# CUAI/Edge-Proposal-Sets

Measured on AMD Instinct MI355X. Metric: candidate edges scored/sec on ogbl-ppa (ppa-like synthetic): Adamic-Adar over the FULL 2-hop non-edge candidate set + top-4M selection, higher is better.
Workload: dtype int64

## Files before the change

edge-proposal-sets_amd/csrc/scan_pieces.hip:

```cpp
#include "eps_common.h"
#include "scan_common.h"
#include <string.h>
#include <atomic>

#define SP_EMPTY 0u
#define SP_MAXP (SP_M + 1)
#define SP_UBITS 8192
#define SP_SB 4
#define SP_PACKED_X8 8u
#define SP_MODE_RATIO 2270u
#define SP_MODE_RATIO_WIDE 8000u
#define SP_BATCH 8
#define SP_G 1
#define SP_LEAN_ROWS 256
#define SP_LEAN_T 256
#define SP_LEAN_G 2
#define SP_LEAN_CHUNK 2048u

typedef short sp_v2s __attribute__((ext_vector_type(2)));

typedef unsigned short sp_v2us __attribute__((ext_vector_type(2)));

struct sp_unit {
    v4i u4;
    v4f a4;
    uint32_t fx;
    int nvalid;
};

template <class Emit>
__device__ __forceinline__ int sp_plan_column(const sp_params &p, int32_t v, int32_t dv, int lane, int32_t my_bound, uint32_t pwk,
                                              int32_t nbk, uint32_t direct_ids, Emit emit)
{
    const uint32_t ek = (uint32_t)eps_wave_incl_scan_dpp((int)pwk) - pwk;
    const bool pk_on = p.ssum != nullptr;
    const uint32_t sv = pk_on ? p.ssum[v] - (p.heads ? (p.heads[v].y < p.ssum[v] ? p.heads[v].y : p.ssum[v]) : 0u) : 0u;
    const uint32_t smk = pk_on ? p.smax[lane <= SP_M ? lane : SP_M] : 0u;
    const int kv = __popcll(__ballot(lane >= 1 && lane < SP_M && my_bound <= v - 1));
    const int32_t hi_k = my_bound < v ? my_bound : v;
    int np = 0, k0 = 0;
    while (k0 <= kv) {
        const int32_t lo = __builtin_amdgcn_readlane(my_bound, k0);
        const uint32_t e0 = (uint32_t)__builtin_amdgcn_readlane((int)ek, k0);
        const bool in = lane > k0 && lane <= kv + 1;
        const int kd = k0 + __popcll(__ballot(in && (uint32_t)(hi_k - lo) <= direct_ids));
        const int32_t nb0 = __builtin_amdgcn_readlane(nbk, k0);
        const int kh = k0 + __popcll(__ballot(in && (ek - e0) + (uint32_t)(nbk - nb0) <= p.piece_paths));
        int kp = k0, kd16 = k0;
        uint32_t ms = 0u;
        if (pk_on) {
            const uint32_t sm0 = (uint32_t)__builtin_amdgcn_readlane((int)smk, k0);
            ms = sv < sm0 ? sv : sm0;
            const uint32_t need_s = (ms >> p.packed_dmax) + (uint32_t)dv + 2u;
            if (need_s < 0x7FFFu) kd16 = k0 + __popcll(__ballot(in && (uint32_t)(hi_k - lo) <= 2u * direct_ids));
            const uint32_t span = (uint32_t)(hi_k - lo);
            const int kb = 32 - __clz((int)((span > 2u ? span : 2u) - 1u));
            const uint32_t cap = kb >= 30 ? 0u : (1u << (31 - kb)) - 1u;
            kp = k0 + __popcll(__ballot(in && (ek - e0) + (uint32_t)(nbk - nb0) <= p.packed_paths && need_s < cap));
            if (p.wide_paths && dv <= p.wide_rows) {
                const int kw = k0 + __popcll(__ballot(in && (ek - e0) <= p.wide_paths));
                kp = kw > kp ? kw : kp;
            }
        }
        int k1;
        uint32_t flag = 0u, pq = 0u;
        const int kdd = kd16 > kd ? kd16 : kd;
        bool take_direct = kdd >= kh && kdd >= kp && kdd > k0;
        if (!take_direct && kdd > k0 && kp > kdd && kp >= kh) {
            const uint32_t pd = (uint32_t)__builtin_amdgcn_readlane((int)ek, kdd) - e0;
            const uint32_t pp = (uint32_t)__builtin_amdgcn_readlane((int)ek, kp) - e0;
            take_direct = (unsigned long long)(pp - pd) * p.mode_ratio < (unsigned long long)pd * pp;
        }
        if (take_direct && kd16 > kd) {
            k1 = kd16;
            flag = 0xC0000000u;
            uint32_t d = 0u;
            while ((ms >> d) + (uint32_t)dv + 2u >= 0x7FFFu) ++d;
            pq = d | (16u << 8);
        } else if (take_direct) {
            k1 = kd;
            flag = 0x80000000u;
        } else if (kp >= kh && kp > k0) {
            k1 = kp;
            flag = 0x40000000u;
            const uint32_t span = (uint32_t)(__builtin_amdgcn_readlane(hi_k, k1) - lo);
            const int kb = 32 - __clz((int)((span > 2u ? span : 2u) - 1u));
            if (p.wide_paths && dv <= p.wide_rows) {
                pq = (uint32_t)(kb < 31 ? kb : 31) << 8;
            } else {
                const uint32_t cap = (1u << (31 - kb)) - 1u;
                uint32_t d = 0u;
                while ((ms >> d) + (uint32_t)dv + 2u >= cap) ++d;
                pq = d | ((uint32_t)kb << 8);
            }
        } else if (kh > k0) {
            k1 = kh;
        } else {
            k1 = k0 + 1;
        }
        const uint32_t sum = (uint32_t)__builtin_amdgcn_readlane((int)ek, k1) - e0;
        if (sum) {
            emit(np, k0, k1, lo, __builtin_amdgcn_readlane(hi_k, k1), sum | flag, pq, __builtin_amdgcn_readlane(nbk, k0),
                 __builtin_amdgcn_readlane(nbk, k1));
            ++np;
        }
        k0 = k1;
    }
    return np;
}

template <int T, bool HV, bool FULL, bool PACK, bool SK = false, bool LEAN = false>
__global__ __launch_bounds__(T, 4) void scan_piece_kernel(sp_params p)
{
    static_assert(!LEAN || (!HV && FULL && PACK && SK), "the lean body serves the main launch's tables only");
    constexpr int G = LEAN ? SP_LEAN_G : SP_G;
    constexpr int ROWS = LEAN ? SP_LEAN_ROWS : T;
    extern __shared__ __attribute__((aligned(16))) uint32_t lds[];
    const int slots = 1 << p.table_bits;
    uint32_t *tkey = lds;
    uint32_t *tval = lds + slots;
    uint4 *r_desc = (uint4 *)(lds + 2 * slots);
    uint32_t *ubits = lds + ((2 * slots + 4 * (ROWS + 1) + 3) & ~3);
    uint16_t *wrank = (uint16_t *)(ubits + SP_UBITS / 32);
    __shared__ unsigned long long s_alloc;
    __shared__ int s_rbase;
    __shared__ int32_t s_pk0[SP_MAXP], s_pk1[SP_MAXP];
    __shared__ int32_t s_plo[SP_MAXP], s_phi[SP_MAXP];
    __shared__ uint32_t s_pinfo[SP_MAXP];
    __shared__ uint32_t s_pq[SP_MAXP];
    __shared__ int32_t s_pna[SP_MAXP], s_pnb[SP_MAXP];
    __shared__ int s_np;
    __shared__ unsigned int s_ticket;
    __shared__ unsigned int s_out_cur, s_out_end;
    __shared__ unsigned int s_fill_lo, s_fill_hi;
    __shared__ unsigned long long s_ncand;
    __shared__ unsigned int s_hot;
    __shared__ uint32_t s_em[SP_EM];

    const int tid = threadIdx.x, lane = tid & 63;
    const int wib = __builtin_amdgcn_readfirstlane(tid >> 6);
    const uint32_t out_cap = p.out->capacity;
    int64_t *__restrict__ out_key = p.out->key;
    float *__restrict__ out_val = p.out->val;
    const uint32_t *__restrict__ rowptr_lo = (const uint32_t *)p.rowptr;
    const __amdgpu_buffer_rsrc_t col_rs = eps_raw_rsrc(p.col, p.col_bytes);
    const __amdgpu_buffer_rsrc_t val_rs = eps_raw_rsrc(HV ? (const void *)p.val : (const void *)p.col, p.col_bytes);
    const uint32_t thr32 = sp_bar_units(p.out->threshold, p.shift, HV);
    const uint32_t direct_ids = 2u * (uint32_t)slots;
    const bool no_bar = !FULL && thr32 <= 1u;
    const bool raw_sums = FULL || p.heads != nullptr;
    const uint32_t chunk = LEAN ? SP_LEAN_CHUNK : no_bar && direct_ids > 8192u ? direct_ids : 8192u;
    const int32_t my_bound = p.bounds[lane <= SP_M ? lane : SP_M];
    if (LEAN && thr32 >= SP_FLAG) {
        if (tid == 0) atomicOr(p.status, 2u);
        return;
    }

    for (int i = tid; i < 2 * slots; i += T) lds[i] = 0u;
    for (int i = tid; i < SP_UBITS / 32; i += T) ubits[i] = 0u;
    for (int i = tid; i < SP_EM; i += T) s_em[i] = 0u;
    if (tid == 0) {
        s_out_cur = 0u;
        s_out_end = 0u;
        s_fill_lo = 0u;
        s_fill_hi = 0u;
        s_alloc = 0ull;
        s_ncand = 0ull;
    }
    bool sketch_seen = false;
    const unsigned int ncol = (unsigned int)p.n_columns;
    const unsigned int batch_from = p.batch_from;
    auto first_of = [&](unsigned int tk) { return tk < batch_from ? tk : batch_from + (tk - batch_from) * SP_BATCH; };
    unsigned int t = blockIdx.x < batch_from ? blockIdx.x : first_of(blockIdx.x);
    unsigned int t_end = t + (blockIdx.x < batch_from ? 1u : SP_BATCH);
    eps_lds_barrier();

    while (t < ncol) {
        const bool last_of_ticket = t + 1u >= t_end || t + 1u >= ncol;
        unsigned int t_next = 0;
        if (tid == 0 && last_of_ticket) t_next = gridDim.x + atomicAdd(p.next_col, 1u);
        int32_t v, dv;
        uint32_t vb;
        uint4 cra = make_uint4(0u, 0u, 0u, 0u), crb = make_uint4(0u, 0u, 0u, 0u);
        if (FULL || p.colrec) {
            cra = p.colrec[2 * (size_t)t];
            crb = p.colrec[2 * (size_t)t + 1];
            v = (int32_t)cra.x;
            vb = cra.y;
            dv = (int32_t)cra.z;
        } else {
            v = p.columns[t];
            vb = rowptr_lo[2 * (size_t)v];
            dv = (int32_t)(rowptr_lo[2 * (size_t)v + 2] - vb);
        }
        const int32_t *__restrict__ vcol = p.col + vb;
        const int32_t *__restrict__ vrev = p.revpos + vb;
        const int rounds = LEAN ? 1 : (dv + T - 1) / T;
        const bool single = LEAN || rounds == 1;
        uint32_t xv = 0u, thr_v = thr32;
        bool bad_head = false;
        if (FULL || p.heads) {
            const uint2 hd = (FULL || p.colrec) ? make_uint2(cra.w, crb.x) : p.heads[v];
            xv = hd.x;
            if (thr32 < SP_FLAG) {
                bad_head = hd.y >= thr32;
                thr_v = thr32 - hd.y;
            }
            if (bad_head && tid == 0) atomicOr(p.status, 4u);
            if ((FULL || p.ssum) && thr32 < SP_FLAG && ((FULL || p.colrec) ? crb.y : p.ssum[v]) < thr32) bad_head = true;
        }
        if (LEAN && dv > ROWS) {
            if (tid == 0) atomicOr(p.status, 2u);
            bad_head = true;
        }
        if (dv > 0 && v > 0 && !bad_head) {
            uint32_t my_w = 0, my_rev = 0, my_base = 0, my_fx = 0;
            uint32_t cut_first = 0u;
            if (PACK && single && tid < dv) {
                const uint4 pa = p.pack[2 * ((size_t)vb + (size_t)tid)];
                my_w = pa.x;
                my_base = pa.y;
                my_fx = pa.z;
                my_rev = pa.w & 0xFFFFu;
                cut_first = pa.w >> 16;
            }
            if (!PACK && single && tid < dv) {
                my_w = (uint32_t)vcol[tid];
                my_rev = (uint32_t)vrev[tid];
            }
            if (!PACK && single && tid < dv) {
                my_base = (FULL || p.rowrec) ? p.rowrec[(size_t)my_w * 32 + 16] : rowptr_lo[2 * (size_t)my_w];
                my_fx = HV ? __builtin_bit_cast(uint32_t, (p.val[vb + tid] * p.node_w[my_w]) * p.up)
                           : ((FULL || p.rowrec) ? p.rowrec[(size_t)my_w * 32 + 17] : p.fx32[my_w]);
            }
            if (!FULL && wib == 0 && !p.plan) {
                const uint32_t pwk = lane < SP_M ? p.wpaths[(size_t)v * SP_M + lane] : 0u;
                const int32_t nbk = lane >= 1 && lane <= SP_M ? (int32_t)p.cuts[(size_t)v * SP_M + lane - 1] : 0;
                const int np = sp_plan_column(p, v, dv, lane, my_bound, pwk, nbk, direct_ids,
                                              [&](int i, int k0, int k1, int32_t lo, int32_t hi, uint32_t info, uint32_t pq, int32_t na, int32_t nb) {
                                                  if (lane == 0) {
                                                      s_pk0[i] = k0;
                                                      s_pk1[i] = k1;
                                                      s_plo[i] = lo;
                                                      s_phi[i] = hi;
                                                      s_pinfo[i] = info;
                                                      s_pq[i] = pq;
                                                      s_pna[i] = na;
                                                      s_pnb[i] = nb;
                                                  }
                                              });
                if (lane == 0) s_np = np;
            } else if (FULL || p.plan) {
                const uint32_t pb = (FULL || p.colrec) ? crb.z : p.pptr[v];
                const int np = (FULL || p.colrec) ? (int)crb.w : (int)(p.pptr[v + 1] - pb);
                if (tid < np) {
                    const uint4 rec = p.plan[pb + (uint32_t)tid];
                    const int k1 = (int)((rec.y >> 8) & 0xFFu);
                    const int32_t bk = p.bounds[k1];
                    s_pinfo[tid] = rec.x;
                    s_pk0[tid] = (int)(rec.y & 0xFFu);
                    s_pk1[tid] = k1;
                    s_pq[tid] = rec.y >> 16;
                    s_pna[tid] = (int32_t)(rec.z & 0xFFFFu);
                    s_pnb[tid] = (int32_t)(rec.z >> 16);
                    s_plo[tid] = (int32_t)rec.w;
                    s_phi[tid] = bk < v ? bk : v;
                }
                if (tid == 0) s_np = np;
            }
            eps_lds_barrier();
            const int np = s_np;
            uint32_t cut_ahead = 0u, seg_from = 0u;
            const uint16_t *__restrict__ cut_tab = (FULL || p.rowrec) ? (const uint16_t *)p.rowrec : p.cuts;
            const size_t cut_ld = (FULL || p.rowrec) ? 64u : (size_t)SP_M;
            const uint16_t *__restrict__ pack16 = (const uint16_t *)p.pack;
            if (PACK) cut_ahead = cut_first;
            else if (single && tid < dv && np > 0) cut_ahead = cut_tab[(size_t)my_w * cut_ld + s_pk1[0] - 1];

            for (int pi = 0; pi < np; ++pi) {
                const int k0 = s_pk0[pi], k1 = s_pk1[pi];
                const int na = s_pna[pi], nb = s_pnb[pi];
                const uint32_t info = s_pinfo[pi];
                if (LEAN && (info >> 30) == 0u) {
                    if (tid == 0) atomicOr(p.status, 2u);
                    continue;
                }
                const bool direct = (info >> 31) != 0u;
                const bool d16 = !HV && (info >> 30) == 3u;
                const bool packed_kind = !HV && (info >> 30) == 1u;
                const bool sketch = LEAN ? packed_kind : SK && packed_kind && single && p.sketch != 0u && thr_v < SP_FLAG;
                const bool packed = !LEAN && packed_kind && !sketch;
                const bool quant = packed || d16;
                const uint32_t ppaths = info & 0x3FFFFFFFu;
                const uint32_t pq = quant ? s_pq[pi] : 0u;
                const uint32_t pk_d = pq & 0xFFu, pk_sb = quant ? 32u - (pq >> 8) : 16u;
                const uint32_t pk_flag = quant ? 1u << (pk_sb - 1u) : 0u;
                const uint32_t pk_thr = thr_v >= SP_FLAG ? 0xFFFFFFFFu : ((thr_v >> pk_d) ? (thr_v >> pk_d) : 1u);
                const int32_t lo_id = s_plo[pi], hi_id = s_phi[pi];
                const uint32_t pkeys = ppaths + (uint32_t)(nb - na);
                int plog = 0;
                if (!LEAN && !direct && !packed && !sketch && pkeys > p.piece_paths) {
                    const uint32_t q = (pkeys + p.piece_paths - 1u) / p.piece_paths;
                    plog = 32 - __clz((int)(q - 1u)) + 1;
                }
                const uint32_t parts = LEAN ? 1u : 1u << plog;
                int bits;
                {
                    const uint32_t per = (pkeys + parts - 1u) >> plog;
                    const int max_bits = packed || sketch ? p.table_bits + 1 : p.table_bits;
                    const int want = per > 1u ? 33 - __clz((int)(per - 1u)) : 1;
                    bits = want < 10 ? 10 : (want > max_bits ? max_bits : want);
                }
                const uint32_t mask = (1u << bits) - 1u;
                const uint32_t span = (uint32_t)(hi_id - lo_id);
                const uint32_t scan_slots = d16 ? (span + 1u) >> 1 : direct ? span : (1u << bits);
                const uint32_t cand_max = direct ? span : (1u << bits);
                if (tid == 0) {
                    s_hot = 0u;
                    uint32_t need = ppaths < cand_max ? ppaths : cand_max;
                    if (!no_bar && need > 1024u) need = 1024u;
                    if (need > chunk) need = chunk;
                    const uint32_t left = s_out_cur < s_out_end ? s_out_end - s_out_cur : 0u;
                    if (left < need) {
                        s_fill_lo = s_out_cur < out_cap ? s_out_cur : out_cap;
                        s_fill_hi = left ? (s_out_end < out_cap ? s_out_end : out_cap) : s_fill_lo;
                        const unsigned long long b64 = atomicAdd(&p.out->count, (unsigned long long)chunk);
                        const uint32_t b = b64 < (unsigned long long)out_cap ? (uint32_t)b64 : out_cap;
                        s_out_cur = b;
                        s_out_end = b + chunk;
                    }
                }
                uint32_t seg_a = 0u, seg_len = 0u;
                if (single && tid < dv) {
                    const uint32_t b = cut_ahead < my_rev ? cut_ahead : my_rev;
                    seg_a = seg_from;
                    seg_len = (uint32_t)tid < xv ? 0u : b - seg_from;
                    seg_from = b;
                    if (pi + 1 < np)
                        cut_ahead = PACK && pi + 1 <= 8 ? pack16[((size_t)vb + (size_t)tid) * 16 + 7 + (pi + 1)]
                                                        : cut_tab[(size_t)my_w * cut_ld + s_pk1[pi + 1] - 1];
                }
                auto emit = [&](uint32_t u, uint32_t sum) {
                    uint32_t pos = atomicAdd(&s_out_cur, 1u);
                    if (pos >= s_out_end) {
                        const unsigned long long q = atomicAdd(&p.out->count, 1ull);
                        pos = q < (unsigned long long)out_cap ? (uint32_t)q : out_cap;
                    }
                    if (pos < out_cap) {
                        out_key[pos] = ((int64_t)v << 32) | (int64_t)u;
                        out_val[pos] = raw_sums ? __builtin_bit_cast(float, sum) : (float)sum * p.scale;
                    }
                };
                for (uint32_t part = 0; part < parts; ++part) {
                    uint32_t new_keys = 0u;
                    for (int j = sketch ? nb : single ? tid : na + tid; j < nb; j += T) {
                        const uint32_t u = single ? my_w : (uint32_t)vcol[j];
                        if (j >= na && (int32_t)u >= lo_id && (int32_t)u < hi_id) {
                            if (d16) {
                                const uint32_t o = u - (uint32_t)lo_id;
                                atomicOr(&lds[o >> 1], 0x8000u << ((o & 1u) << 4));
                            } else if (direct) {
                                lds[u - (uint32_t)lo_id] = SP_FLAG;
                            } else if (packed) {
                                const uint32_t mix = sp_mix(u);
                                uint32_t h = mix >> (32 - bits);
                                const uint32_t st = ((mix >> 7) | 1u) & mask;
                                const uint32_t word = ((u - (uint32_t)lo_id) << pk_sb) | pk_flag;
                                for (uint32_t tries = 0; tries <= mask; ++tries) {
                                    if (atomicCAS(&lds[h], 0u, word) == 0u) break;
                                    h = (h + st) & mask;
                                }
                            } else if (!LEAN) {
                                const uint32_t mix = sp_mix(u);
                                if ((mix & (parts - 1u)) == part) {
                                    uint32_t h = mix >> (32 - bits);
                                    const uint32_t st = ((mix >> 7) | 1u) & mask;
                                    for (uint32_t tries = 0; tries <= mask; ++tries) {
                                        if (atomicCAS(&tkey[h], SP_EMPTY, u + 1u) == SP_EMPTY) {
                                            tval[h] = SP_FLAG;
                                            break;
                                        }
                                        h = (h + st) & mask;
                                    }
                                }
                            }
                        }
                    }
                    for (int r = 0; r < rounds; ++r) {
                        const int j = r * T + tid;
                        uint32_t w = my_w, rev = my_rev, base = my_base, fx = my_fx;
                        uint32_t len = 0u, a = 0u;
                        if (single) {
                            a = seg_a;
                            len = seg_len;
                        } else if (j < dv) {
                            w = (uint32_t)vcol[j];
                            rev = (uint32_t)vrev[j];
                            base = (FULL || p.rowrec) ? p.rowrec[(size_t)w * 32 + 16] : rowptr_lo[2 * (size_t)w];
                            fx = HV ? __builtin_bit_cast(uint32_t, (p.val[vb + j] * p.node_w[w]) * p.up)
                                    : ((FULL || p.rowrec) ? p.rowrec[(size_t)w * 32 + 17] : p.fx32[w]);
                            const uint16_t *crow = cut_tab + (size_t)w * cut_ld;
                            uint32_t b = crow[k1 - 1];
                            if (k0 > 0) a = crow[k0 - 1];
                            a = a < rev ? a : rev;
                            b = b < rev ? b : rev;
                            len = (uint32_t)j < xv ? 0u : b - a;
                        }
                        const int units = (int)((len + 3u) >> 2);
                        const int flag = units > 0 ? 1 : 0;
                        const int incl_c = eps_wave_incl_scan_dpp(units | (flag << 24));
                        const int incl = incl_c & 0xFFFFFF, incl_f = (int)((uint32_t)incl_c >> 24);
                        unsigned long long got = 0ull;
                        if (lane == 63) got = atomicAdd(&s_alloc, ((unsigned long long)(uint32_t)incl << 32) | (unsigned long long)(uint32_t)incl_f);
                        const int woff = __builtin_amdgcn_readlane((int)(got >> 32), 63);
                        const int woff_f = __builtin_amdgcn_readlane((int)(uint32_t)got, 63);
                        const uint32_t a_u = (uint32_t)(incl - units + woff);
                        if (flag) {
                            const int d = incl_f - 1 + woff_f;
                            r_desc[d] = make_uint4(base + a, len, quant ? (fx + ((1u << pk_d) - 1u)) >> pk_d : fx, a_u);
                            if (a_u < (uint32_t)SP_UBITS) atomicOr(&ubits[a_u >> 5], 1u << (a_u & 31u));
                        }
                        eps_lds_barrier();
                        if (s_fill_hi > s_fill_lo) {
                            const uint32_t f0 = s_fill_lo, f1 = s_fill_hi;
                            for (uint32_t i = f0 + (uint32_t)tid; i < f1; i += T) {
                                out_key[i] = -1;
                                out_val[i] = -__builtin_inff();
                            }
                        }
                        int total = (int)(s_alloc >> 32);
                        if (LEAN && total > SP_UBITS) {
                            if (tid == 0) atomicOr(p.status, 2u);
                            total = SP_UBITS;
                        }
                        for (uint32_t ulo = 0; ulo < (uint32_t)total && (!LEAN || ulo == 0u); ulo += SP_UBITS) {
                            const uint32_t uhi = ulo + SP_UBITS < (uint32_t)total ? ulo + SP_UBITS : (uint32_t)total;
                            if (ulo > 0u) {
                                for (int i = tid; i < SP_UBITS / 32; i += T) ubits[i] = 0u;
                                if (tid == 0) s_rbase = 0;
                                eps_lds_barrier();
                                const unsigned long long before = __ballot(flag && a_u + (uint32_t)units <= ulo);
                                if (lane == 0 && before) atomicAdd(&s_rbase, __popcll(before));
                                if (flag && a_u + (uint32_t)units > ulo && a_u < uhi) {
                                    const uint32_t pos = (a_u > ulo ? a_u : ulo) - ulo;
                                    atomicOr(&ubits[pos >> 5], 1u << (pos & 31));
                                }
                                eps_lds_barrier();
                            }
                            const int rbase = ulo > 0u ? s_rbase : 0;
                            {
                                const uint4 b4 = *(const uint4 *)(ubits + 4 * lane);
                                const int c0 = __popc(b4.x), c1 = c0 + __popc(b4.y), c2 = c1 + __popc(b4.z), c3 = c2 + __popc(b4.w);
                                const int ex = eps_wave_incl_scan_dpp(c3) - c3;
                                uint2 pk;
                                pk.x = (uint32_t)ex | ((uint32_t)(ex + c0) << 16);
                                pk.y = (uint32_t)(ex + c1) | ((uint32_t)(ex + c2) << 16);
                                *(uint2 *)(wrank + 4 * lane) = pk;
                                asm volatile("s_waitcnt lgkmcnt(0)" ::: "memory");
                            }
                        auto fetch_group = [&](int it0, sp_unit (&f)[G]) {
                            int lo[G];
#pragma unroll
                            for (int q = 0; q < G; ++q) {
                                const uint32_t sr = (uint32_t)((it0 + q) * T + tid);
                                const uint32_t wd = sr < SP_UBITS ? sr >> 5 : 0u;
                                const uint32_t bits = ubits[wd];
                                const int rk = (int)wrank[wd];
                                lo[q] = rbase + rk + __popc(bits & ((2u << (sr & 31u)) - 1u)) - 1;
                                lo[q] = lo[q] < 0 ? 0 : lo[q];
                            }
#pragma unroll
                            for (int q = 0; q < G; ++q) {
                                const int s = (int)ulo + (it0 + q) * T + tid;
// ... 107 lines not shown
                                        }
                                    }
                                    if (++tries > 4u * (mask + 2u)) {
                                        if (have || pend) atomicOr(p.status, 2u);
                                        have = false;
                                        pend = 0u;
                                    }
                                }
                            } else if (!LEAN) {
                                constexpr int E = 4 * G;
                                uint32_t key[E], h[E], mixv[E];
                                uint32_t pend = 0u;
#pragma unroll
                                for (int q = 0; q < G; ++q) pend |= ((1u << f[q].nvalid) - 1u) << (4 * q);
#pragma unroll
                                for (int i = 0; i < E; ++i) {
                                    const uint32_t id = (uint32_t)f[i >> 2].u4[i & 3];
                                    mixv[i] = sp_mix(id);
                                    key[i] = id + 1u;
                                    h[i] = mixv[i] >> (32 - bits);
                                }
                                if (parts > 1u) {
#pragma unroll
                                    for (int i = 0; i < E; ++i)
                                        if ((mixv[i] & (parts - 1u)) != part) pend &= ~(1u << i);
                                }
                                uint32_t old[E], pfx[E];
#pragma unroll
                                for (int i = 0; i < E; ++i) pfx[i] = path_fx(f[i >> 2], i & 3);
#pragma unroll
                                for (int i = 0; i < E; ++i)
                                    if (pend & (1u << i)) old[i] = atomicCAS(&tkey[h[i]], SP_EMPTY, key[i]);
#pragma unroll
                                for (int i = 0; i < E; ++i)
                                    if ((pend & (1u << i)) && (old[i] == SP_EMPTY || old[i] == key[i])) {
                                        atomicAdd(&tval[h[i]], pfx[i]);
                                        pend &= ~(1u << i);
                                        new_keys += old[i] == SP_EMPTY ? 1u : 0u;
                                    }
                                uint32_t ch = 0u, cstep = 0u, ckey = 0u, cfx = 0u, tries = 0u;
                                bool have = false;
                                while (__ballot(have || pend != 0u)) {
                                    if (!have && pend != 0u) {
                                        const int e = __ffs((int)pend) - 1;
                                        pend &= pend - 1u;
                                        uint32_t m = mixv[0];
                                        ch = h[0];
                                        ckey = key[0];
                                        cfx = pfx[0];
#pragma unroll
                                        for (int i = 1; i < E; ++i)
                                            if (e == i) {
                                                m = mixv[i];
                                                ch = h[i];
                                                ckey = key[i];
                                                cfx = pfx[i];
                                            }
                                        cstep = ((m >> 7) | 1u) & mask;
                                        have = true;
                                    }
                                    if (have) {
                                        ch = (ch + cstep) & mask;
                                        const uint32_t o = atomicCAS(&tkey[ch], SP_EMPTY, ckey);
                                        if (o == SP_EMPTY || o == ckey) {
                                            atomicAdd(&tval[ch], cfx);
                                            new_keys += o == SP_EMPTY ? 1u : 0u;
                                            have = false;
                                        }
                                    }
                                    if (++tries > 4u * (mask + 2u)) {
                                        if (have || pend) atomicOr(p.status, 2u);
                                        have = false;
                                        pend = 0u;
                                    }
                                }
                            }
                        };
                        {
                            const int n_iter = (int)(uhi - ulo + T - 1) / T;
                            sp_unit fa[G], fb[G];
                            fetch_group(0, fa);
                            if (n_iter <= G) {
                                consume_group(fa);
                            } else {
                                for (int it0 = 0; it0 < n_iter; it0 += 2 * G) {
                                    fetch_group(it0 + G, fb);
                                    consume_group(fa);
                                    fetch_group(it0 + 2 * G, fa);
                                    consume_group(fb);
                                }
                            }
                        }
                        if (sketch) {
                            if (tid == 0 && !sketch_seen) atomicOr(p.status, 16u);
                            sketch_seen = true;
                            eps_lds_barrier();
                            const uint32_t half = 1u << (bits - 1);
                            {
                                uint32_t mx = 0u;
                                for (uint32_t i = 4u * (uint32_t)tid; i < half; i += 4u * T) {
                                    const uint4 a4 = *(const uint4 *)(lds + i);
                                    const uint32_t m01 = a4.x > a4.y ? a4.x : a4.y, m23 = a4.z > a4.w ? a4.z : a4.w;
                                    const uint32_t m = m01 > m23 ? m01 : m23;
                                    mx = m > mx ? m : mx;
                                }
                                if (__ballot(mx >= thr_v) && lane == 0) s_hot = 1u;
                            }
                            eps_lds_barrier();
                            if (s_hot) {
                            const int n_iter = (int)(uhi - ulo + T - 1) / T;
                            auto report = [&](uint32_t u, uint32_t est) {
                                int a = na, b = nb;
                                while (a < b) {
                                    const int mid = (a + b) >> 1;
                                    if (vcol[mid] < (int32_t)u) a = mid + 1; else b = mid;
                                }
                                if (a < nb && vcol[a] == (int32_t)u) return;
                                const uint32_t em_mask = (p.sketch >> 1 ? p.sketch >> 1 : (uint32_t)SP_EM) - 1u;
                                uint32_t h = (sp_mix(u) >> 9) & em_mask;
                                for (uint32_t tries = 0; tries <= em_mask; ++tries) {
                                    const uint32_t old = atomicCAS(&s_em[h], 0u, u + 1u);
                                    if (old == 0u) {
                                        emit(u, est);
                                        return;
                                    }
                                    if (old == u + 1u) return;
                                    h = (h + 1u) & em_mask;
                                }
                                atomicOr(p.status, 8u);
                            };
                            auto look = [&](const sp_unit (&f)[G]) {
                                uint32_t est[4 * G];
#pragma unroll
                                for (int i = 0; i < 4 * G; ++i) {
                                    const uint32_t id = (uint32_t)f[i >> 2].u4[i & 3];
                                    const uint32_t ea = lds[sp_mix(id) >> (33 - bits)], eb = lds[half + (sp_mix2(id) >> (33 - bits))];
                                    est[i] = ea < eb ? ea : eb;
                                }
#pragma unroll
                                for (int i = 0; i < 4 * G; ++i)
                                    if ((i & 3) < f[i >> 2].nvalid && est[i] >= thr_v) report((uint32_t)f[i >> 2].u4[i & 3], est[i]);
                            };
                            sp_unit fa[G], fb[G];
                            fetch_group(0, fa);
                            if (n_iter <= G) {
                                look(fa);
                            } else {
                                for (int it0 = 0; it0 < n_iter; it0 += 2 * G) {
                                    fetch_group(it0 + G, fb);
                                    look(fa);
                                    fetch_group(it0 + 2 * G, fa);
                                    look(fb);
                                }
                            }
                            }
                        }
                            if (!LEAN && uhi < (uint32_t)total) eps_lds_barrier();
                        }
                        eps_lds_barrier();
                        for (int i = tid; i < SP_UBITS / 32; i += T) ubits[i] = 0u;
                        if (tid == 0) {
                            s_alloc = 0ull;
                            s_fill_hi = 0u;
                        }
                        if (r + 1 < rounds) eps_lds_barrier();
                    }
                    const int thr_s = thr_v >= SP_FLAG ? 0x7FFFFFFF : (int)thr_v;
                    if (d16) {
                        const int thr_h = pk_thr >= 0x8000u ? 0x7FFFFFFF : (int)(pk_thr << 16);
                        sp_v2us pc16 = (sp_v2us)(0);
                        uint32_t ones = 0x00010001u;
                        asm("" : "+v"(ones));
                        const uint32_t n4 = (scan_slots + 3u) & ~3u;
                        for (uint32_t i0 = 0; i0 < n4; i0 += 4u * SP_SB * T) {
                            uint4 s4[SP_SB];
#pragma unroll
                            for (int b = 0; b < SP_SB; ++b) {
                                const uint32_t i = i0 + 4u * T * b + 4u * tid;
                                s4[b] = i < n4 ? *(const uint4 *)(lds + i) : make_uint4(0u, 0u, 0u, 0u);
                            }
#pragma unroll
                            for (int b = 0; b < SP_SB; ++b) {
                                const uint32_t i = i0 + 4u * T * b + 4u * tid;
                                if (i < n4) *(uint4 *)(lds + i) = make_uint4(0u, 0u, 0u, 0u);
                                const uint32_t wv[4] = {s4[b].x, s4[b].y, s4[b].z, s4[b].w};
#pragma unroll
                                for (int e = 0; e < 4; ++e) {
                                    const sp_v2s pos = __builtin_elementwise_max(__builtin_bit_cast(sp_v2s, wv[e]), (sp_v2s)(0));
                                    pc16 += __builtin_elementwise_min(__builtin_bit_cast(sp_v2us, pos), __builtin_bit_cast(sp_v2us, ones));
                                }
                                int x[8];
#pragma unroll
                                for (int e = 0; e < 4; ++e) {
                                    x[2 * e] = (int)(wv[e] << 16);
                                    x[2 * e + 1] = (int)(wv[e] & 0xFFFF0000u);
                                }
                                int m = x[0];
#pragma unroll
                                for (int e = 1; e < 8; ++e) m = x[e] > m ? x[e] : m;
                                if (m >= thr_h) {
#pragma unroll
                                    for (int e = 0; e < 8; ++e)
                                        if (x[e] >= thr_h) emit((uint32_t)lo_id + 2u * i + e, ((uint32_t)x[e] >> 16) << pk_d);
                                }
                            }
                        }
                        new_keys += (uint32_t)pc16.x + (uint32_t)pc16.y;
                    } else if (direct) {
                        const uint32_t n4 = (scan_slots + 3u) & ~3u;
                        for (uint32_t i0 = 0; i0 < n4; i0 += 4u * SP_SB * T) {
                            uint4 s4[SP_SB];
#pragma unroll
                            for (int b = 0; b < SP_SB; ++b) {
                                const uint32_t i = i0 + 4u * T * b + 4u * tid;
                                s4[b] = i < n4 ? *(const uint4 *)(lds + i) : make_uint4(0u, 0u, 0u, 0u);
                            }
#pragma unroll
                            for (int b = 0; b < SP_SB; ++b) {
                                const uint32_t i = i0 + 4u * T * b + 4u * tid;
                                if (i < n4) *(uint4 *)(lds + i) = make_uint4(0u, 0u, 0u, 0u);
                                const int sv[4] = {(int)s4[b].x, (int)s4[b].y, (int)s4[b].z, (int)s4[b].w};
#pragma unroll
                                for (int e = 0; e < 4; ++e) new_keys += sv[e] > 0 ? 1u : 0u;
                                const int m01 = sv[0] > sv[1] ? sv[0] : sv[1], m23 = sv[2] > sv[3] ? sv[2] : sv[3];
                                if ((m01 > m23 ? m01 : m23) >= thr_s) {
#pragma unroll
                                    for (int e = 0; e < 4; ++e)
                                        if (sv[e] >= thr_s) emit((uint32_t)lo_id + i + e, (uint32_t)sv[e]);
                                }
                            }
                        }
                    } else if (sketch) {
                        for (uint32_t i = 4u * (uint32_t)tid; i < scan_slots; i += 4u * T) *(uint4 *)(lds + i) = make_uint4(0u, 0u, 0u, 0u);
                        for (int i = tid; i < SP_EM; i += T) s_em[i] = 0u;
                    } else if (packed) {
                        const uint32_t kb = 32u - pk_sb;
                        const int thr_p = pk_thr >= pk_flag ? 0x7FFFFFFF : (int)(pk_thr << kb);
                        for (uint32_t i0 = 0; i0 < scan_slots; i0 += 4u * SP_SB * T) {
                            uint4 s4[SP_SB];
#pragma unroll
                            for (int b = 0; b < SP_SB; ++b) {
                                const uint32_t i = i0 + 4u * T * b + 4u * tid;
                                s4[b] = i < scan_slots ? *(const uint4 *)(lds + i) : make_uint4(0u, 0u, 0u, 0u);
                            }
#pragma unroll
                            for (int b = 0; b < SP_SB; ++b) {
                                const uint32_t i = i0 + 4u * T * b + 4u * tid;
                                if (i < scan_slots) *(uint4 *)(lds + i) = make_uint4(0u, 0u, 0u, 0u);
                                const uint32_t sv[4] = {s4[b].x, s4[b].y, s4[b].z, s4[b].w};
                                const int x[4] = {(int)(sv[0] << kb), (int)(sv[1] << kb), (int)(sv[2] << kb), (int)(sv[3] << kb)};
                                const int m01 = x[0] > x[1] ? x[0] : x[1], m23 = x[2] > x[3] ? x[2] : x[3];
                                if ((m01 > m23 ? m01 : m23) >= thr_p) {
#pragma unroll
                                    for (int e = 0; e < 4; ++e)
                                        if (x[e] >= thr_p) emit((uint32_t)lo_id + (sv[e] >> pk_sb), ((uint32_t)x[e] >> kb) << pk_d);
                                }
                            }
                        }
                    } else if (!LEAN) {
                        for (uint32_t i0 = 0; i0 < scan_slots; i0 += 4u * SP_SB * T) {
                            uint4 s4[SP_SB];
#pragma unroll
                            for (int b = 0; b < SP_SB; ++b) {
                                const uint32_t i = i0 + 4u * T * b + 4u * tid;
                                s4[b] = i < scan_slots ? *(const uint4 *)(tval + i) : make_uint4(0u, 0u, 0u, 0u);
                            }
#pragma unroll
                            for (int b = 0; b < SP_SB; ++b) {
                                const uint32_t i = i0 + 4u * T * b + 4u * tid;
                                const int sv[4] = {(int)s4[b].x, (int)s4[b].y, (int)s4[b].z, (int)s4[b].w};
                                const int m01 = sv[0] > sv[1] ? sv[0] : sv[1], m23 = sv[2] > sv[3] ? sv[2] : sv[3];
                                if ((m01 > m23 ? m01 : m23) >= thr_s) {
#pragma unroll
                                    for (int e = 0; e < 4; ++e)
                                        if (sv[e] >= thr_s) emit(tkey[i + e] - 1u, (uint32_t)sv[e]);
                                }
                                if (i < scan_slots) {
                                    *(uint4 *)(tkey + i) = make_uint4(0u, 0u, 0u, 0u);
                                    *(uint4 *)(tval + i) = make_uint4(0u, 0u, 0u, 0u);
                                }
                            }
                        }
                    }
                    {
                        const uint32_t upto = (uint32_t)eps_wave_incl_scan_dpp((int)new_keys);
                        if (lane == 63 && upto) atomicAdd(&s_ncand, (unsigned long long)upto);
                    }
                    eps_lds_barrier();
                }
            }
        }
        if (!last_of_ticket) {
            ++t;
            eps_lds_barrier();
            continue;
        }
        if (tid == 0) s_ticket = t_next;
        eps_lds_barrier();
        const unsigned int tk = s_ticket;
        eps_lds_barrier();
        t = first_of(tk);
        t_end = t + (tk < batch_from ? 1u : SP_BATCH);
    }
    {
        const uint32_t f0 = s_out_cur < out_cap ? s_out_cur : out_cap, f1 = s_out_end < out_cap ? s_out_end : out_cap;
        for (uint32_t i = f0 + (uint32_t)tid; i < f1; i += T) {
            out_key[i] = -1;
            out_val[i] = -__builtin_inff();
        }
    }
    if (tid == 0 && s_ncand) atomicAdd(&p.out->n_candidates, s_ncand);
}

static const int sp_threads_of[3] = {512, 1024, 256}, sp_bits_of[3] = {13, 14, 12}, sp_per_cu[3] = {2, 1, 4};
#define SP_VARIANT_GEOM(v) ((v) & 0xFF)
#define SP_VARIANT_DMAX(v) ((((v) >> 8) & 0xFF) - 1)
#define SP_VARIANT_WIDE(v) (((v) >> 24) & 1)
#define SP_VARIANT_SKETCH(v) (((v) >> 16) & 0xFF)

static void sp_plan_geometry(sp_params &p, const uint16_t *cuts, const uint32_t *wpaths, const uint32_t *ssum, const uint32_t *smax,
                             const int32_t *bounds, int64_t n_nodes, int32_t shift, int32_t variant, int32_t dmax_arg)
{
    const int bits = sp_bits_of[variant];
    p.cuts = cuts;
    p.wpaths = wpaths;
    p.bounds = bounds;
    p.n_nodes = (int32_t)n_nodes;
    p.table_bits = bits;
    p.piece_paths = (1u << bits) / 2u;
    p.ssum = ssum;
    p.smax = smax;
    p.packed_paths = (SP_PACKED_X8 << bits) / 8u;
    p.packed_dmax = shift > 8 ? (shift - 8 < 24 ? shift - 8 : 24) : 0;
    if (dmax_arg >= 0 && dmax_arg < p.packed_dmax) p.packed_dmax = dmax_arg;
    p.mode_ratio = SP_MODE_RATIO;
    p.shift = shift;
}

__global__ __launch_bounds__(256) void sp_plan_kernel(sp_params p, const int64_t *__restrict__ rowptr, uint32_t direct_ids,
                                                      uint32_t *__restrict__ pcount, const uint32_t *__restrict__ pptr, uint4 *__restrict__ out,
                                                      uint32_t *__restrict__ d_used)
{
    const int lane = threadIdx.x & 63;
    const int64_t v = (int64_t)blockIdx.x * 4 + (threadIdx.x >> 6);
    if (v >= p.n_nodes) return;
    const int32_t dv = (int32_t)(rowptr[v + 1] - rowptr[v]);
    int np = 0;
    if (dv > 0 && v > 0) {
        const int32_t my_bound = p.bounds[lane <= SP_M ? lane : SP_M];
        const uint32_t pwk = lane < SP_M ? p.wpaths[(size_t)v * SP_M + lane] : 0u;
        const int32_t nbk = lane >= 1 && lane <= SP_M ? (int32_t)p.cuts[(size_t)v * SP_M + lane - 1] : 0;
        const uint32_t pb = out ? pptr[v] : 0u;
        np = sp_plan_column(p, (int32_t)v, dv, lane, my_bound, pwk, nbk, direct_ids,
                            [&](int i, int k0, int k1, int32_t lo, int32_t hi, uint32_t info, uint32_t pq, int32_t na, int32_t nb) {
                                if (out && lane == 0) {
                                    out[pb + (uint32_t)i] = make_uint4(info, (uint32_t)k0 | ((uint32_t)k1 << 8) | (pq << 16),
                                                                       (uint32_t)na | ((uint32_t)nb << 16), (uint32_t)lo);
                                    if (d_used && (info & 0x40000000u) && (pq & 0xFFu) > __atomic_load_n(d_used, __ATOMIC_RELAXED))
                                        atomicMax(d_used, pq & 0xFFu);
                                }
                            });
    }
    if (!out && lane == 0) pcount[v] = (uint32_t)np;
}

extern "C" int eps_scan_plan(const int64_t *rowptr, const uint16_t *cuts, const uint32_t *wpaths, const uint32_t *ssum_or_null,
                             const uint32_t *smax_or_null, const uint32_t *heads_or_null, const int32_t *bounds, int64_t n_nodes,
                             int32_t shift, int32_t variant, uint32_t *pcount, const uint32_t *pptr_or_null, uint32_t *plan_or_null,
                             uint32_t *d_used_or_null, void *stream)
{
    EPS_REQUIRE(n_nodes >= 0 && n_nodes < (1ll << 31), "eps_scan_plan: bad size");
    if (d_used_or_null && hipMemsetAsync(d_used_or_null, 0, sizeof(uint32_t), (hipStream_t)stream) != hipSuccess) {
        eps_set_error("eps_scan_plan: cannot clear d_used");
        return EPS_ELAUNCH;
    }
    if (n_nodes == 0) return EPS_OK;
    EPS_REQUIRE(rowptr && cuts && wpaths && bounds, "eps_scan_plan: null pointer");
    EPS_REQUIRE((ssum_or_null == nullptr) == (smax_or_null == nullptr), "eps_scan_plan: ssum and smax come together");
    EPS_REQUIRE((pptr_or_null == nullptr) == (plan_or_null == nullptr), "eps_scan_plan: pptr and plan come together");
    EPS_REQUIRE(pptr_or_null || pcount, "eps_scan_plan: nowhere to put the counts");
    const int32_t dmax_arg = SP_VARIANT_DMAX(variant);
    const bool wide_arg = SP_VARIANT_WIDE(variant) != 0;
    variant = SP_VARIANT_GEOM(variant);
    EPS_REQUIRE(shift >= 0 && shift <= 40 && variant >= 0 && variant <= 2, "eps_scan_plan: bad shift / variant");
    EPS_REQUIRE(((uintptr_t)plan_or_null & 15) == 0, "eps_scan_plan: plan must be 16-byte aligned");
    sp_params p;
    memset(&p, 0, sizeof p);
    sp_plan_geometry(p, cuts, wpaths, ssum_or_null, smax_or_null, bounds, n_nodes, shift, variant, dmax_arg);
    if (wide_arg && ssum_or_null) {
        p.wide_paths = 2u << sp_bits_of[variant];
        if (p.wide_paths > SP_UBITS) p.wide_paths = SP_UBITS;
        p.wide_rows = sp_threads_of[variant];
        p.mode_ratio = SP_MODE_RATIO_WIDE;
    }
    p.heads = (const uint2 *)heads_or_null;
    hipLaunchKernelGGL(sp_plan_kernel, dim3((unsigned)((n_nodes + 3) / 4)), dim3(256), 0, (hipStream_t)stream, p, rowptr,
                       2u << sp_bits_of[variant], pcount, pptr_or_null, (uint4 *)plan_or_null, d_used_or_null);
    EPS_CHECK_LAUNCH("eps_scan_plan");
    return EPS_OK;
}

__global__ __launch_bounds__(256) void sp_rewalk_kernel(const uint4 *__restrict__ plan, int64_t n_rec, uint32_t cap,
                                                        unsigned long long *__restrict__ out)
{
    unsigned long long re = 0ull, all = 0ull;
    for (int64_t i = (int64_t)blockIdx.x * blockDim.x + threadIdx.x; i < n_rec; i += (int64_t)gridDim.x * blockDim.x) {
        const uint4 r = plan[i];
        const uint32_t paths = r.x & 0x3FFFFFFFu;
        all += paths;
        if ((r.x >> 30) == 0u) {
            const uint32_t keys = paths + ((r.z >> 16) - (r.z & 0xFFFFu));
            if (keys > cap) {
                const uint32_t q = (keys + cap - 1u) / cap;
                const uint32_t parts = 2u << (32 - __clz((int)(q - 1u)));
                re += (unsigned long long)paths * (parts - 1u);
            }
        }
    }
#pragma unroll
    for (int d = 32; d >= 1; d >>= 1) {
        re += __shfl_xor(re, d);
        all += __shfl_xor(all, d);
    }
    if ((threadIdx.x & 63) == 0) {
        if (re) atomicAdd(&out[0], re);
        if (all) atomicAdd(&out[1], all);
    }
}

extern "C" int eps_scan_plan_rewalk(const uint32_t *plan, int64_t n_rec, int32_t variant, unsigned long long *out2, void *stream)
{
    EPS_REQUIRE(n_rec >= 0 && out2 && variant >= 0 && variant <= 2, "eps_scan_plan_rewalk: bad argument");
    hipStream_t s = (hipStream_t)stream;
    if (hipMemsetAsync(out2, 0, 2 * sizeof(unsigned long long), s) != hipSuccess) {
        eps_set_error("eps_scan_plan_rewalk: cannot clear the result");
        return EPS_ELAUNCH;
    }
    if (n_rec == 0) return EPS_OK;
    EPS_REQUIRE(plan && ((uintptr_t)plan & 15) == 0, "eps_scan_plan_rewalk: plan must be 16-byte aligned");
    int64_t blocks = (n_rec + 255) / 256;
    if (blocks > 2048) blocks = 2048;
    hipLaunchKernelGGL(sp_rewalk_kernel, dim3((unsigned)blocks), dim3(256), 0, s, (const uint4 *)plan, n_rec,
                       (1u << sp_bits_of[variant]) / 2u, out2);
    EPS_CHECK_LAUNCH("eps_scan_plan_rewalk");
    return EPS_OK;
}

static size_t sp_lds_bytes(int bits, int rows) { return ((size_t)(2 << bits) + 4 * (size_t)(rows + 1) + 8) * 4 + (SP_UBITS / 32) * 6 + 32; }

extern "C" int eps_scan_lean_blocks_per_cu(void)
{
    static std::atomic<int> cached{0};
    int per_cu = cached.load();
    if (per_cu < 1) {
        const void *lean = (const void *)scan_piece_kernel<SP_LEAN_T, false, true, true, true, true>;
        const size_t lds = sp_lds_bytes(sp_bits_of[2], SP_LEAN_ROWS);
        if (hipFuncSetAttribute(lean, hipFuncAttributeMaxDynamicSharedMemorySize, (int)lds) != hipSuccess ||
            hipOccupancyMaxActiveBlocksPerMultiprocessor(&per_cu, lean, SP_LEAN_T, lds) != hipSuccess || per_cu < 1) {
            eps_set_error("eps_scan_screen: no occupancy figure for the lean body at %zu bytes of LDS", lds);
            return EPS_ELAUNCH;
        }
        cached.store(per_cu);
    }
    return per_cu;
}

static int sp_launch(const int64_t *rowptr, const int32_t *col, const float *val, const int32_t *revpos, const uint32_t *fx32,
                     const float *node_w, const uint16_t *cuts, const uint32_t *wpaths, const uint32_t *ssum, const uint32_t *smax,
                     const uint32_t *pptr, const uint32_t *plan, const uint32_t *heads, const uint32_t *rowrec, const uint32_t *pack,
                     const int32_t *bounds, int64_t n_nodes, int64_t nnz, const int32_t *columns, const uint32_t *colrec, int64_t n_columns, int64_t batch_from,
                     int64_t lean_from, int64_t lean_batch_from, int64_t light_from, int32_t shift, int32_t variant, eps_survivors *out,
                     uint32_t *status, void *stream)
{
    EPS_REQUIRE(n_nodes >= 0 && n_columns >= 0 && nnz >= 0, "eps_scan_screen: negative size");
    EPS_REQUIRE(status, "eps_scan_screen: null pointer");
    hipStream_t s = (hipStream_t)stream;
    if (hipMemsetAsync(status, 0, sizeof(uint32_t), s) != hipSuccess) {
        eps_set_error("eps_scan_screen: cannot clear the status word");
        return EPS_ELAUNCH;
    }
    if (n_columns == 0 || n_nodes == 0) return EPS_OK;
    EPS_REQUIRE(rowptr && col && revpos && cuts && wpaths && bounds && columns && out, "eps_scan_screen: null pointer");
    EPS_REQUIRE(nnz < (1ll << 30), "eps_scan_screen: col[] is addressed with 32-bit byte offsets (nnz < 2^30)");
    EPS_REQUIRE(n_nodes < (1ll << 31) && n_columns < (1ll << 31), "eps_scan_screen: too many nodes / columns");
    const uint32_t sketch_arg = (uint32_t)SP_VARIANT_SKETCH(variant);
    EPS_REQUIRE(!SP_VARIANT_WIDE(variant) || ((sketch_arg & 1u) && plan && !val && SP_VARIANT_GEOM(variant) == 2),
                "eps_scan_screen: a plan with wide packed pieces (variant bit 24) is for sketch launches (bit 16) of the 256-thread geometry");
    const int32_t dmax_arg = SP_VARIANT_DMAX(variant);
    variant = SP_VARIANT_GEOM(variant);
    EPS_REQUIRE(shift >= 0 && shift <= 40 && variant >= 0 && variant <= 2, "eps_scan_screen: bad shift / variant");
    EPS_REQUIRE(((uintptr_t)cuts & 15) == 0, "eps_scan_screen: cuts must be 16-byte aligned");
    EPS_REQUIRE(((uintptr_t)colrec & 15) == 0 && ((uintptr_t)rowrec & 127) == 0, "eps_scan_screen: misaligned column / row records");
    EPS_REQUIRE(!colrec || plan, "eps_scan_screen: column records come with the plan table they were built from");
    EPS_REQUIRE((pptr == nullptr) == (plan == nullptr) && ((uintptr_t)plan & 15) == 0, "eps_scan_screen: pptr and plan come together, 16-byte aligned");
    const int T = sp_threads_of[variant], bits = sp_bits_of[variant];
    if (light_from < 0 || light_from > n_columns) light_from = n_columns;
    if (lean_from < 0 || lean_from > light_from) lean_from = light_from;
    const int64_t n_main = lean_from, n_lean = light_from - lean_from;
    unsigned int *counter = nullptr;
    const int rc = eps_take_counter(&counter, s, "eps_scan_screen");
    if (rc) return rc;
    sp_params p;
    memset(&p, 0, sizeof p);
    p.rowptr = rowptr;
    p.col = col;
    p.revpos = revpos;
    p.fx32 = fx32;
    p.val = val;
    p.node_w = node_w;
    p.up = ldexpf(1.0f, shift) * (1.0f + ldexpf(1.0f, -20));
    sp_plan_geometry(p, cuts, wpaths, ssum, smax, bounds, n_nodes, shift, variant, dmax_arg);
    p.pptr = pptr;
    p.plan = (const uint4 *)plan;
    p.heads = (const uint2 *)heads;
    p.rowrec = rowrec;
    p.pack = (const uint4 *)pack;
    p.colrec = (const uint4 *)colrec;
    p.columns = columns;
    p.n_columns = (int32_t)n_main;
    p.batch_from = batch_from < 0 || batch_from > n_main ? (uint32_t)n_main : (uint32_t)batch_from;
    p.sketch = val || !(sketch_arg & 1u) ? 0u : sketch_arg;
    p.col_bytes = (uint32_t)(nnz * 4);
    p.scale = ldexpf(1.0f, -shift);
    p.next_col = counter;
    p.out = out;
    p.status = status;
    int64_t blocks = (int64_t)eps_num_cus() * sp_per_cu[variant];
    if (blocks > n_main) blocks = n_main;
    const size_t lds = sp_lds_bytes(bits, T);
    void (*kern)(sp_params) =
        val ? (variant == 0 ? scan_piece_kernel<512, true, false, false> : variant == 1 ? scan_piece_kernel<1024, true, false, false>
                                                                                       : scan_piece_kernel<256, true, false, false>)
            : (variant == 0 ? scan_piece_kernel<512, false, false, false> : variant == 1 ? scan_piece_kernel<1024, false, false, false>
                                                                                         : scan_piece_kernel<256, false, false, false>);
    const bool full = !val && variant == 2 && plan && colrec && rowrec && heads && ssum;
    EPS_REQUIRE(!pack || full, "eps_scan_screen: the column pack serves the main launch only (variant 2, plan, records, heads, sum bounds)");
    if (full) kern = pack ? scan_piece_kernel<256, false, true, true> : scan_piece_kernel<256, false, true, false>;
    if (p.sketch && variant == 2)
        kern = full ? (pack ? scan_piece_kernel<256, false, true, true, true> : scan_piece_kernel<256, false, true, false, true>)
                    : scan_piece_kernel<256, false, false, false, true>;
    else
        p.sketch = 0u;
    if (hipFuncSetAttribute((const void *)kern, hipFuncAttributeMaxDynamicSharedMemorySize, (int)lds) != hipSuccess) {
        eps_set_error("eps_scan_screen: cannot reserve %zu bytes of LDS", lds);
        return EPS_ELAUNCH;
    }
    EPS_REQUIRE(n_main == n_columns || (full && pack && p.sketch),
                "eps_scan_screen: a lean or light zone comes with the main launch's tables (plan, records, heads, pack) and sketch pieces (bit 16)");
    if (n_main > 0) {
        hipLaunchKernelGGL(kern, dim3((unsigned)blocks), dim3(T), lds, s, p);
        EPS_CHECK_LAUNCH("eps_scan_screen");
    }
    if (n_lean > 0) {
        sp_params q = p;
        const int rc2 = eps_take_counter(&q.next_col, s, "eps_scan_screen");
        if (rc2) return rc2;
        q.columns = columns + lean_from;
        q.colrec = (const uint4 *)colrec + 2 * lean_from;
        q.n_columns = (int32_t)n_lean;
        q.batch_from = lean_batch_from < 0 || lean_batch_from > n_lean ? (uint32_t)n_lean : (uint32_t)lean_batch_from;
        void (*lean)(sp_params) = scan_piece_kernel<SP_LEAN_T, false, true, true, true, true>;
        const size_t lds_lean = sp_lds_bytes(bits, SP_LEAN_ROWS);
        const int per_cu = eps_scan_lean_blocks_per_cu();
        if (per_cu < 1) return per_cu;
        if (hipFuncSetAttribute((const void *)lean, hipFuncAttributeMaxDynamicSharedMemorySize, (int)lds_lean) != hipSuccess) {
            eps_set_error("eps_scan_screen: cannot reserve %zu bytes of LDS", lds_lean);
            return EPS_ELAUNCH;
        }
        int64_t nb = (int64_t)eps_num_cus() * (per_cu < sp_per_cu[variant] ? per_cu : sp_per_cu[variant]);
        if (nb > n_lean) nb = n_lean;
        hipLaunchKernelGGL(lean, dim3((unsigned)nb), dim3(SP_LEAN_T), lds_lean, s, q);
        EPS_CHECK_LAUNCH("eps_scan_screen");
    }
    p.n_columns = (int32_t)n_columns;
    return sl_launch(p, (uint32_t)light_from, (uint32_t)n_columns, 12, s);
}

extern "C" int eps_scan_screen(const int64_t *rowptr, const int32_t *col, const int32_t *revpos, const uint32_t *fx32,
                               const uint16_t *cuts, const uint32_t *wpaths, const uint32_t *ssum_or_null,
                               const uint32_t *smax_or_null, const uint32_t *pptr_or_null, const uint32_t *plan_or_null,
                               const uint32_t *heads_or_null, const uint32_t *rowrec_or_null, const uint32_t *pack_or_null,
                               const int32_t *bounds, int64_t n_nodes, int64_t nnz,
                               const int32_t *columns, const uint32_t *colrec_or_null, int64_t n_columns, int64_t batch_from,
                               int64_t lean_from, int64_t lean_batch_from, int64_t light_from, int32_t shift, int32_t variant,
                               eps_survivors *out, uint32_t *status, void *stream)
{
    EPS_REQUIRE(!pack_or_null || (plan_or_null && rowrec_or_null && ((uintptr_t)pack_or_null & 15) == 0),
                "eps_scan_screen: the column pack comes with the plan table and the row records it was built from, 16-byte aligned");
    EPS_REQUIRE(n_columns == 0 || n_nodes == 0 || fx32, "eps_scan_screen: null pointer");
    EPS_REQUIRE((ssum_or_null == nullptr) == (smax_or_null == nullptr), "eps_scan_screen: ssum and smax come together");
    EPS_REQUIRE(!heads_or_null || plan_or_null, "eps_scan_screen: a head table comes with the plan table built for it");
    return sp_launch(rowptr, col, nullptr, revpos, fx32, nullptr, cuts, wpaths, ssum_or_null, smax_or_null, pptr_or_null,
                     plan_or_null, heads_or_null, rowrec_or_null, pack_or_null, bounds, n_nodes, nnz, columns, colrec_or_null, n_columns,
                     batch_from, lean_from, lean_batch_from, light_from, shift, variant, out, status, stream);
}

extern "C" int eps_scan_screen_weighted(const int64_t *rowptr, const int32_t *col, const float *val, const int32_t *revpos,
                                        const float *node_w, const uint16_t *cuts, const uint32_t *wpaths,
                                        const int32_t *bounds, int64_t n_nodes, int64_t nnz, const int32_t *columns,
                                        int64_t n_columns, int32_t shift, int32_t variant, eps_survivors *out, uint32_t *status,
                                        void *stream)
{
    EPS_REQUIRE(n_columns == 0 || n_nodes == 0 || (val && node_w), "eps_scan_screen_weighted: null pointer");
    return sp_launch(rowptr, col, val, revpos, nullptr, node_w, cuts, wpaths, nullptr, nullptr, nullptr, nullptr, nullptr, nullptr, nullptr,
                     bounds, n_nodes, nnz, columns, nullptr, n_columns, n_columns, n_columns, 0, n_columns, shift, variant, out, status, stream);
}

__global__ void scan_pieces_warm_kernel() {}
extern "C" void eps_warm_scan_pieces(void *stream) { hipLaunchKernelGGL(scan_pieces_warm_kernel, dim3(1), dim3(1), 0, (hipStream_t)stream); }
```

Baseline: 1464 billion.

## Fuse main and lean scan launches into one persistent kernel

Moves the kernel body into a device function templated on first/last phase and adds a fused kernel. When both zones exist, each block runs the main-zone body and then the lean-zone body, sharing LDS state and the output fill and candidate-count flush, so one launch replaces two. This removes a launch boundary and the tail-drain gap between the two kernels. In exchange the main zone now runs with the lean launch's grid size rather than its own block count, and the lean zone inherits the main zone's output cursor. Shared variables become file-scope statics.

Result: faster. 1487 billion, median of 6 (+1.6%).

```diff
diff --git a/edge-proposal-sets_amd/csrc/scan_pieces.hip b/edge-proposal-sets_amd/csrc/scan_pieces.hip
--- a/edge-proposal-sets_amd/csrc/scan_pieces.hip
+++ b/edge-proposal-sets_amd/csrc/scan_pieces.hip
@@ -109,8 +109,23 @@
     return np;
 }
 
-template <int T, bool HV, bool FULL, bool PACK, bool SK = false, bool LEAN = false>
-__global__ __launch_bounds__(T, 4) void scan_piece_kernel(sp_params p)
+static __shared__ unsigned long long s_alloc;
+static __shared__ int s_rbase;
+static __shared__ int32_t s_pk0[SP_MAXP], s_pk1[SP_MAXP];
+static __shared__ int32_t s_plo[SP_MAXP], s_phi[SP_MAXP];
+static __shared__ uint32_t s_pinfo[SP_MAXP];
+static __shared__ uint32_t s_pq[SP_MAXP];
+static __shared__ int32_t s_pna[SP_MAXP], s_pnb[SP_MAXP];
+static __shared__ int s_np;
+static __shared__ unsigned int s_ticket;
+static __shared__ unsigned int s_out_cur, s_out_end;
+static __shared__ unsigned int s_fill_lo, s_fill_hi;
+static __shared__ unsigned long long s_ncand;
+static __shared__ unsigned int s_hot;
+static __shared__ uint32_t s_em[SP_EM];
+
+template <int T, bool HV, bool FULL, bool PACK, bool SK, bool LEAN, bool FIRST = true, bool LAST = true>
+__device__ __forceinline__ void sp_body(const sp_params p)
 {
     static_assert(!LEAN || (!HV && FULL && PACK && SK), "the lean body serves the main launch's tables only");
     constexpr int G = LEAN ? SP_LEAN_G : SP_G;
@@ -122,20 +137,6 @@
     uint4 *r_desc = (uint4 *)(lds + 2 * slots);
     uint32_t *ubits = lds + ((2 * slots + 4 * (ROWS + 1) + 3) & ~3);
     uint16_t *wrank = (uint16_t *)(ubits + SP_UBITS / 32);
-    __shared__ unsigned long long s_alloc;
-    __shared__ int s_rbase;
-    __shared__ int32_t s_pk0[SP_MAXP], s_pk1[SP_MAXP];
-    __shared__ int32_t s_plo[SP_MAXP], s_phi[SP_MAXP];
-    __shared__ uint32_t s_pinfo[SP_MAXP];
-    __shared__ uint32_t s_pq[SP_MAXP];
-    __shared__ int32_t s_pna[SP_MAXP], s_pnb[SP_MAXP];
-    __shared__ int s_np;
-    __shared__ unsigned int s_ticket;
-    __shared__ unsigned int s_out_cur, s_out_end;
-    __shared__ unsigned int s_fill_lo, s_fill_hi;
-    __shared__ unsigned long long s_ncand;
-    __shared__ unsigned int s_hot;
-    __shared__ uint32_t s_em[SP_EM];
 
     const int tid = threadIdx.x, lane = tid & 63;
     const int wib = __builtin_amdgcn_readfirstlane(tid >> 6);
@@ -151,24 +152,26 @@
     const bool raw_sums = FULL || p.heads != nullptr;
     const uint32_t chunk = LEAN ? SP_LEAN_CHUNK : no_bar && direct_ids > 8192u ? direct_ids : 8192u;
     const int32_t my_bound = p.bounds[lane <= SP_M ? lane : SP_M];
+    bool no_zone = false;
     if (LEAN && thr32 >= SP_FLAG) {
         if (tid == 0) atomicOr(p.status, 2u);
-        return;
+        if (FIRST && LAST) return;
+        no_zone = true;
     }
 
     for (int i = tid; i < 2 * slots; i += T) lds[i] = 0u;
     for (int i = tid; i < SP_UBITS / 32; i += T) ubits[i] = 0u;
     for (int i = tid; i < SP_EM; i += T) s_em[i] = 0u;
     if (tid == 0) {
-        s_out_cur = 0u;
-        s_out_end = 0u;
+        if (FIRST) s_out_cur = 0u;
+        if (FIRST) s_out_end = 0u;
         s_fill_lo = 0u;
         s_fill_hi = 0u;
         s_alloc = 0ull;
-        s_ncand = 0ull;
+        if (FIRST) s_ncand = 0ull;
     }
     bool sketch_seen = false;
-    const unsigned int ncol = (unsigned int)p.n_columns;
+    const unsigned int ncol = no_zone ? 0u : (unsigned int)p.n_columns;
     const unsigned int batch_from = p.batch_from;
     auto first_of = [&](unsigned int tk) { return tk < batch_from ? tk : batch_from + (tk - batch_from) * SP_BATCH; };
     unsigned int t = blockIdx.x < batch_from ? blockIdx.x : first_of(blockIdx.x);
@@ -882,6 +885,7 @@
         t = first_of(tk);
         t_end = t + (tk < batch_from ? 1u : SP_BATCH);
     }
+    if (!LAST) return;
     {
         const uint32_t f0 = s_out_cur < out_cap ? s_out_cur : out_cap, f1 = s_out_end < out_cap ? s_out_end : out_cap;
         for (uint32_t i = f0 + (uint32_t)tid; i < f1; i += T) {
@@ -890,6 +894,19 @@
         }
     }
     if (tid == 0 && s_ncand) atomicAdd(&p.out->n_candidates, s_ncand);
+}
+
+template <int T, bool HV, bool FULL, bool PACK, bool SK = false, bool LEAN = false>
+__global__ __launch_bounds__(T, 4) void scan_piece_kernel(sp_params p)
+{
+    sp_body<T, HV, FULL, PACK, SK, LEAN>(p);
+}
+
+__global__ __launch_bounds__(256, 4) void scan_fused_kernel(sp_params p, sp_params q)
+{
+    static_assert(SP_LEAN_T == 256 && SP_LEAN_ROWS == 256, "both bodies run on the same threads and the same LDS layout");
+    sp_body<256, false, true, true, true, false, true, false>(p);
+    sp_body<256, false, true, true, true, true, false, true>(q);
 }
 
 static const int sp_threads_of[3] = {512, 1024, 256}, sp_bits_of[3] = {13, 14, 12}, sp_per_cu[3] = {2, 1, 4};
@@ -1038,6 +1055,22 @@
         if (hipFuncSetAttribute(lean, hipFuncAttributeMaxDynamicSharedMemorySize, (int)lds) != hipSuccess ||
             hipOccupancyMaxActiveBlocksPerMultiprocessor(&per_cu, lean, SP_LEAN_T, lds) != hipSuccess || per_cu < 1) {
             eps_set_error("eps_scan_screen: no occupancy figure for the lean body at %zu bytes of LDS", lds);
+            return EPS_ELAUNCH;
+        }
+        cached.store(per_cu);
+    }
+    return per_cu;
+}
+
+static int sp_fused_blocks_per_cu(void)
+{
+    static std::atomic<int> cached{0};
+    int per_cu = cached.load();
+    if (per_cu < 1) {
+        const size_t lds = sp_lds_bytes(sp_bits_of[2], SP_LEAN_ROWS);
+        if (hipFuncSetAttribute((const void *)scan_fused_kernel, hipFuncAttributeMaxDynamicSharedMemorySize, (int)lds) != hipSuccess ||
+            hipOccupancyMaxActiveBlocksPerMultiprocessor(&per_cu, (const void *)scan_fused_kernel, SP_LEAN_T, lds) != hipSuccess || per_cu < 1) {
+            eps_set_error("eps_scan_screen: no occupancy figure for the fused kernel at %zu bytes of LDS", lds);
             return EPS_ELAUNCH;
         }
         cached.store(per_cu);
@@ -1127,10 +1160,6 @@
     }
     EPS_REQUIRE(n_main == n_columns || (full && pack && p.sketch),
                 "eps_scan_screen: a lean or light zone comes with the main launch's tables (plan, records, heads, pack) and sketch pieces (bit 16)");
-    if (n_main > 0) {
-        hipLaunchKernelGGL(kern, dim3((unsigned)blocks), dim3(T), lds, s, p);
-        EPS_CHECK_LAUNCH("eps_scan_screen");
-    }
     if (n_lean > 0) {
         sp_params q = p;
         const int rc2 = eps_take_counter(&q.next_col, s, "eps_scan_screen");
@@ -1139,17 +1168,23 @@
         q.colrec = (const uint4 *)colrec + 2 * lean_from;
         q.n_columns = (int32_t)n_lean;
         q.batch_from = lean_batch_from < 0 || lean_batch_from > n_lean ? (uint32_t)n_lean : (uint32_t)lean_batch_from;
-        void (*lean)(sp_params) = scan_piece_kernel<SP_LEAN_T, false, true, true, true, true>;
+        const bool fused = n_main > 0;
+        const void *fn = fused ? (const void *)scan_fused_kernel : (const void *)scan_piece_kernel<SP_LEAN_T, false, true, true, true, true>;
         const size_t lds_lean = sp_lds_bytes(bits, SP_LEAN_ROWS);
-        const int per_cu = eps_scan_lean_blocks_per_cu();
+        const int per_cu = fused ? sp_fused_blocks_per_cu() : eps_scan_lean_blocks_per_cu();
         if (per_cu < 1) return per_cu;
-        if (hipFuncSetAttribute((const void *)lean, hipFuncAttributeMaxDynamicSharedMemorySize, (int)lds_lean) != hipSuccess) {
+        if (hipFuncSetAttribute(fn, hipFuncAttributeMaxDynamicSharedMemorySize, (int)lds_lean) != hipSuccess) {
             eps_set_error("eps_scan_screen: cannot reserve %zu bytes of LDS", lds_lean);
             return EPS_ELAUNCH;
         }
         int64_t nb = (int64_t)eps_num_cus() * (per_cu < sp_per_cu[variant] ? per_cu : sp_per_cu[variant]);
-        if (nb > n_lean) nb = n_lean;
-        hipLaunchKernelGGL(lean, dim3((unsigned)nb), dim3(SP_LEAN_T), lds_lean, s, q);
+        const int64_t most = n_main > n_lean ? n_main : n_lean;
+        if (nb > most) nb = most;
+        if (fused) hipLaunchKernelGGL(scan_fused_kernel, dim3((unsigned)nb), dim3(SP_LEAN_T), lds_lean, s, p, q);
+        else hipLaunchKernelGGL((scan_piece_kernel<SP_LEAN_T, false, true, true, true, true>), dim3((unsigned)nb), dim3(SP_LEAN_T), lds_lean, s, q);
+        EPS_CHECK_LAUNCH("eps_scan_screen");
+    } else if (n_main > 0) {
+        hipLaunchKernelGGL(kern, dim3((unsigned)blocks), dim3(T), lds, s, p);
         EPS_CHECK_LAUNCH("eps_scan_screen");
     }
     p.n_columns = (int32_t)n_columns;
```
